# nubcico/EAV

Hardware: AMD Instinct MI355X
Metric: EEGNet training samples/sec (fwd+CE+bwd+Adam), whole job (higher is better)
Workload: dtype f32; 1 GPU; EEGNet_tor(5, Chans=30, Samples=10000, kernLength=300, F1=8, D=8, F2=64) train step on x[64,1,30,10000] fp32 per GPU (BASELINE.json configs[1]); global_batch=64, per_gpu_batch=64, parallelism=dp1

## Files before the change

### eav_amd/_lib.py

```python
from __future__ import annotations

import ctypes as C
import os

_HERE = os.path.dirname(os.path.abspath(__file__))
LIB_PATH = os.environ.get("EAV_LIB_PATH") or os.path.join(_HERE, "libeav_hip.so")


class EavError(RuntimeError):
    pass


_p = C.c_void_p
_i = C.c_int
_i64 = C.c_int64
_u64 = C.c_uint64
_f = C.c_float
_d = C.c_double

SIGNATURES = {
    "eav_reduce_partials": [_p, _i, _i64, _i, _f, _p, _p],
    "eav_bn_finalize": [_p, _i, _i, _d, _p, _p, _p, _p, _i, _f, _f, _p, _p, _p, _p, _p],
    "eav_bn_bwd_finalize": [_p, _i, _i, _d, _i, _p, _p, _p, _p, _p],
    "eav_reduce_and_bn_bwd_finalize": [_p, _i, _i64, _i, _p, _p, _i, _i, _d, _i, _p, _p, _p, _p, _p, _i, _i, _d, _i, _p, _p, _p,
                                       _p, _p],
    "eav_renorm_rows": [_p, _i, _i, _f, _p],
    "eav_renorm_rows2": [_p, _i, _i, _p, _i, _i, _f, _p],
    "eav_eegnet_step_prologue": [_p, _p, _p, _p, _p, _p, _p, _p],
    "eav_eegnet_fir_fwd": [_p, _p, _p, _p, _i, _i, _i, _i, _p],
    "eav_eegnet_fir_wgrad": [_p, _p, _p, _p, _p, _i, _i, _i, _i, _p],
    "eav_eegnet_fir_fwd_indexed": [_p, _p, _p, _p, _p, _i, _i, _i, _i, _p],
    "eav_eegnet_fir_fwd_fft": [_p, _p, _p, _p, _p, _i, _i, _i, _i, _p],
    "eav_eegnet_fir_wgrad_fft": [_p, _p, _p, _p, _p, _p, _p, _i, _i, _i, _i, _p],
    "eav_eegnet_fir_wgrad_indexed": [_p, _p, _p, _p, _p, _p, _i, _i, _i, _i, _p],
    "eav_eegnet_dw_fwd": [_p, _p, _p, _p, _p, _i, _i, _i, _p],
    "eav_eegnet_dw_fwd_pool_eval": [_p, _p, _p, _p, _p, _p, _p, _i, _i, _i, _p],
    "eav_eegnet_dw_bwd": [_p, _p, _p, _p, _p, _p, _p, _i, _i, _i, _p],
    "eav_eegnet_dw_bwd_fused": [_p, _p, _p, _p, _p, _p, _p, _p, _p, _i, _i, _i, _f, _u64, _p, _p, _p],
    "eav_eegnet_dw_bwd_fused_eval": [_p, _p, _p, _p, _p, _p, _p, _p, _p, _p, _i, _i, _i, _f, _u64, _p, _p, _p],
    "eav_bn_elu_pool_fwd": [_p, _p, _p, _i, _i, _i, _i, _f, _u64, _p, _p, _p],
    "eav_bn_elu_pool_bwd_reduce": [_p, _p, _p, _p, _i, _i, _i, _i, _f, _u64, _p, _p, _p],
    "eav_bn_elu_pool_bwd_apply": [_p, _p, _p, _p, _p, _i, _i, _i, _i, _f, _u64, _p, _p, _p],
    "eav_bn_elu_pool_bwd_eval": [_p, _p, _p, _p, _p, _i, _i, _i, _i, _f, _u64, _p, _p, _p],
    "eav_conv64_prep_weights": [_p, _p, _p, _p],
    "eav_conv64_fwd": [_p, _p, _p, _p, _i, _i, _i, _p],
    "eav_conv64_wgrad": [_p, _p, _p, _i, _i, _i, _p],
    "eav_conv64_fft_fwd": [_p, _p, _p, _p, _p, _i, _i, _i, _p],
    "eav_conv64_fft_wgrad": [_p, _p, _p, _i, _i, _p],
    "eav_dense_softmax_fwd": [_p, _p, _p, _p, _p, _i, _i, _i, _p],
    "eav_dense_softmax_bwd": [_p, _p, _p, _p, _p, _p, _p, _i, _i, _i, _p],
    "eav_ce_fwd_bwd": [_p, _p, _p, _p, _p, _p, _i, _i, _p],
    "eav_scale_by_scalar": [_p, _p, _i64, _p],
    "eav_adam_step": [_p, _p, _p, _p, _i64, _f, _f, _f, _f, _f, _i64, _i, _p, _p],
    "eav_counter_inc": [_p, _p],
    "eav_counter_inc4": [_p, _p, _p, _p, _p],
    "eav_step_begin": [_p, _p, _p, _p, _p, _p, _p, _p, _i, _p],
    "eav_gather_rows": [_p, _p, _p, _i, _i64, _p],
    "eav_gather_i64": [_p, _p, _p, _i, _p],
    "eav_gemm_f32": [_p, _p, _p, _i, _i, _i, _i, _i, _i, _i, _i, _i, _i, _i64, _i64, _i64, _i64, _i64, _i64, _f, _p,
                     _i, _p, _p, _i, _i, _p],
    "eav_gemm_f32_splitk": [_p, _p, _p, _p, _i, _i, _i, _i, _i, _i, _i, _p],
    "eav_sp_absmax": [_p, _i, _i, _i64, _p, _p],
    "eav_sp_convert": [_p, _i, _i, _i64, _p, _p, _p, _p],
    "eav_sp_convert_gelu": [_p, _i, _i, _i64, _p, _p, _p, _p],
    "eav_sp_convert_colsum": [_p, _i, _i, _i64, _p, _p, _p, _p, _p],
    "eav_layernorm_fwd_amax": [_p, _p, _p, _p, _p, _p, _i, _i, _f, _p, _p],
    "eav_layernorm_bwd_amax": [_p, _p, _p, _p, _p, _p, _i, _p, _i, _i, _p, _p],
    "eav_layernorm_bwd_planes": [_p, _p, _p, _p, _p, _p, _i, _p, _i, _i, _p, _p, _p, _p, _p, _p],
    "eav_layernorm_bwd_bound": [_p, _p, _p, _p, _p, _i, _i, _p, _p],
    "eav_gelu_bwd_amax": [_p, _p, _i64, _p, _p],
    "eav_gemm_sp": [_p, _p, _p, _p, _p, _i, _i, _i, _i, _i, _i64, _i64, _f, _p, _i, _p, _p, _i, _i, _p, _p],
    "eav_gemm_sp_x1": [_p, _p, _p, _p, _p, _i, _i, _i, _i, _i, _i64, _i64, _f, _p, _i, _p, _p, _i, _i, _p, _p],
    "eav_gemm_sp_splitk_x1": [_p, _p, _p, _p, _p, _p, _i, _i, _i, _i, _p],
    "eav_gemm_sp_splitk_x2": [_p, _p, _p, _p, _p, _p, _i, _i, _i, _i, _p],
    "eav_gemm_sp_ex": [_p, _p, _p, _p, _p, _i, _i, _i, _i, _i, _i64, _i64, _f, _p, _i, _p, _p, _i, _i, _p, _p, _p, _p, _i, _p],
    "eav_colnorm_max": [_p, _i, _i, _i64, _p, _p],
    "eav_norm_max_multi": [_p, _i, _i, _p],
    "eav_sp_bound_scale": [_p, _p, _p, _f, _p],
    "eav_gemm_sp_planes": [_p, _p, _p, _p, _p, _i, _i, _i, _i, _i, _i64, _i64, _f, _p, _i, _p, _p, _i, _i, _p, _p, _p, _p],
    "eav_layernorm_fwd_planes": [_p, _p, _p, _p, _p, _p, _p, _p, _i, _i, _f, _p],
    "eav_sp_refresh_planes": [_p, _i, _i, _i, _p],
# ... 206 lines not shown
```

### eav_amd/csrc/eav_common.h

```cpp
#pragma once
#include <hip/hip_runtime.h>
#include <stdint.h>

#define EAV_OK 0
#define EAV_EINVAL (-1)
#define EAV_ELAUNCH (-2)
#define EAV_EUNSUPPORTED (-3)

int eav_set_error(int code, const char* fmt, ...);

#define EAV_REQUIRE(cond, ...)                                   \
  do {                                                           \
    if (!(cond)) return eav_set_error(EAV_EINVAL, __VA_ARGS__);  \
  } while (0)

#define EAV_CHECK_LAUNCH(name)                                                        \
  do {                                                                                \
    hipError_t e__ = hipGetLastError();                                               \
    if (e__ != hipSuccess)                                                            \
      return eav_set_error(EAV_ELAUNCH, "%s: %s", name, hipGetErrorString(e__));      \
  } while (0)

typedef float f32x4 __attribute__((ext_vector_type(4)));
typedef float f32x16 __attribute__((ext_vector_type(16)));

static inline int cdiv(int a, int b) { return (a + b - 1) / b; }
static inline int64_t cdiv64(int64_t a, int64_t b) { return (a + b - 1) / b; }

#ifdef EAV_ABL_ELU
__device__ __forceinline__ float elu_f(float v) { return v > 0.f ? v : 0.5f * v; }
#elif defined(EAV_ELU_LIBM)
__device__ __forceinline__ float elu_f(float v) {
  const float e = expm1f(fminf(v, 0.f));
  return v <= 0.f ? e : v;
}
#else
__device__ __forceinline__ float expm1_neg(float x) {
#pragma clang fp contract(off)
  const float t = __builtin_fmaf(x, 1.4426950408889634f, 12582912.f);
  const float n = t - 12582912.f;
  float r = __builtin_fmaf(n, -0.693145751953125f, x);
  r = __builtin_fmaf(n, -1.42860682030941723212e-6f, r);
  float q = 1.394644962e-03f;
  q = __builtin_fmaf(q, r, 8.366583847e-03f);
  q = __builtin_fmaf(q, r, 4.166628048e-02f);
  q = __builtin_fmaf(q, r, 1.666654348e-01f);
  q = __builtin_fmaf(q, r, 0.5f);
  const float p = __builtin_fmaf(r * r, q, r);
  const float s = __uint_as_float((__float_as_uint(t) << 23) + 0x3f800000u);
  return __builtin_fmaf(p, s, s - 1.f);
}
__device__ __forceinline__ float elu_f(float v) {
  const float e = expm1_neg(__builtin_amdgcn_fmed3f(v, -17.5f, 0.f));
  return v <= 0.f ? e : v;
}
#endif
__device__ __forceinline__ float elu_grad_from_out(float v, float a) { return v > 0.f ? 1.f : a + 1.f; }

__device__ __forceinline__ float wave_sum(float v) {
#pragma unroll
  for (int o = 32; o > 0; o >>= 1) v += __shfl_xor(v, o, 64);
  return v;
}
__device__ __forceinline__ float half_sum(float v) {
#pragma unroll
  for (int o = 16; o > 0; o >>= 1) v += __shfl_xor(v, o, 64);
  return v;
}

template <int NV>
__device__ __forceinline__ void block_sum_256(float (&v)[NV], float* red) {
  const int lane = threadIdx.x & 63, wave = threadIdx.x >> 6;
#pragma unroll
  for (int k = 0; k < NV; ++k) {
    float s = wave_sum(v[k]);
    if (lane == 0) red[wave * NV + k] = s;
  }
  __syncthreads();
  if (threadIdx.x < NV) {
    v[0] = red[threadIdx.x] + red[NV + threadIdx.x] + red[2 * NV + threadIdx.x] + red[3 * NV + threadIdx.x];
  }
  __syncthreads();
}

#define EAV_SLOT_SHARD(i) (32 * ((i) & 63))
#define EAV_SLOT_SIGMA 2048
#define EAV_SLOT_ISIGMA 2049
#define EAV_SLOT_BMAX 2080
#define EAV_SLOT_BEXP 3104
#define EAV_SLOT_NBLK 1024
// ... 45 lines not shown
```

### eav_amd/csrc/eegnet_block.hip

```cpp
#include "eav_common.h"
#include "../../include/eav_hip.h"

namespace {

constexpr int F1 = 8, DD = 8, CHMAX = 32;

__device__ __forceinline__ void ld4(const float* p, int i, int n, bool vec, float (&v)[4]) {
  if (vec && i + 3 < n) {
    float4 a = *reinterpret_cast<const float4*>(p + i);
    v[0] = a.x; v[1] = a.y; v[2] = a.z; v[3] = a.w;
  } else {
#pragma unroll
    for (int e = 0; e < 4; ++e) v[e] = (i + e < n) ? p[i + e] : 0.f;
  }
}
__device__ __forceinline__ void ld4s(const float* p, int i, int n, bool vec, float (&v)[4]) {
  if (vec && i + 3 < n) {
    const f32x4 a = __builtin_nontemporal_load(reinterpret_cast<const f32x4*>(p + i));
    v[0] = a[0]; v[1] = a[1]; v[2] = a[2]; v[3] = a[3];
  } else {
#pragma unroll
    for (int e = 0; e < 4; ++e) v[e] = (i + e < n) ? p[i + e] : 0.f;
  }
}
// ... 184 lines not shown
  block_sum_256<2>(st, red);
  if (threadIdx.x < 2) part[(int64_t)b * 2 * CH + threadIdx.x * CH + ch] = st[0];
}

template <int P>
__global__ __launch_bounds__(256) void pool_bwd_apply_kernel(const float* __restrict__ dp,
                                                             const float* __restrict__ u,
                                                             const float* __restrict__ bn,
                                                             const float* __restrict__ m12, float* __restrict__ du,
                                                             int CH, int T, float drop_p, uint64_t seed_in,
    const uint8_t* __restrict__ mask, const uint64_t* __restrict__ seed_dev, float* __restrict__ part) {
  const uint64_t seed = dropout_seed(seed_in, seed_dev);
  __shared__ float red[8];
  const int row = blockIdx.x, ch = row % CH;
  const float mean = bn[ch], invstd = bn[CH + ch], sc = bn[2 * CH + ch], sh = bn[3 * CH + ch];
  const float m1 = m12 ? m12[ch] : 0.f, m2 = m12 ? m12[CH + ch] : 0.f;
  float st[2] = {0.f, 0.f};
  const int To = T / P;
  const float* src = u + (int64_t)row * T;
  float* dst = du + (int64_t)row * T;
  const bool vec = (T & 3) == 0;
  for (int q = threadIdx.x; q < (T + 3) / 4; q += 256) {
    const int t = 4 * q;
    const int to = t / P;
    float go = 0.f;
    if (to < To) {
      const uint64_t oi = (uint64_t)row * To + to;
      go = dp[oi] * (1.0f / P) * dropout_mult_row(drop_p, seed, mask, oi, (uint64_t)row);
    }
    float v[4], o[4];
    ld4(src, t, T, vec, v);
#pragma unroll
    for (int e = 0; e < 4; ++e) {
      const float pre = sc * v[e] + sh;
      const float g = go * elu_grad_from_out(pre, elu_f(pre));
      o[e] = sc * (g - m1 - (v[e] - mean) * invstd * m2);
      if (t + e < T) {
        st[0] += g;
        st[1] += g * ((v[e] - mean) * invstd);
      }
    }
    st4(dst, t, T, vec, o);
  }
  if (part) {
    block_sum_256<2>(st, red);
    if (threadIdx.x < 2) part[(int64_t)(row / CH) * 2 * CH + threadIdx.x * CH + ch] = st[0];
  }
}

template <int CTRL, int BANK_MASK>
__device__ __forceinline__ float dpp_f(float old, float src) {
  return __int_as_float(__builtin_amdgcn_update_dpp(__float_as_int(old), __float_as_int(src), CTRL, 0xf, BANK_MASK, false));
}

template <int CTRL, int ROW_MASK, bool BOUND>
__device__ __forceinline__ float dpp_row(float src) {
  return __int_as_float(__builtin_amdgcn_update_dpp(0, __float_as_int(src), CTRL, ROW_MASK, 0xf, BOUND));
}
__device__ __forceinline__ float wave_total_dpp(float a) {
  a += dpp_row<0x111, 0xf, true>(a);
  a += dpp_row<0x112, 0xf, true>(a);
  a += dpp_row<0x114, 0xf, true>(a);
  a += dpp_row<0x118, 0xf, true>(a);
  a += dpp_row<0x142, 0xa, false>(a);
  a += dpp_row<0x143, 0xc, false>(a);
  return __int_as_float(__builtin_amdgcn_readlane(__float_as_int(a), 63));
}

struct DwFuse {
  const float* z; const float* dp2; const float* bn2;
  float drop_p; uint64_t seed; const uint8_t* mask; const uint64_t* seed_dev;
  float* part2;
// ... 320 lines not shown
```

### eav_amd/csrc/eegnet_conv64_fft.hip

```cpp
#include <algorithm>

#include "eav_common.h"
#include "../../include/eav_hip.h"

namespace {

constexpr int NCH = 64, KT = 16, NB = 64, LV = NB - KT + 1;
typedef float v2f __attribute__((ext_vector_type(2)));
typedef __attribute__((address_space(3))) void* lds_ptr_t;
constexpr float C64[50] = {1.0f, 0.995184727f, 0.98078528f, 0.956940336f, 0.923879533f, 0.881921264f, 0.831469612f, 0.773010453f, 0.707106781f, 0.634393284f, 0.555570233f, 0.471396737f, 0.382683432f, 0.290284677f, 0.195090322f, 0.0980171403f, 0.0f, -0.0980171403f, -0.195090322f, -0.290284677f, -0.382683432f, -0.471396737f, -0.555570233f, -0.634393284f, -0.707106781f, -0.773010453f, -0.831469612f, -0.881921264f, -0.923879533f, -0.956940336f, -0.98078528f, -0.995184727f, -1.0f, -0.995184727f, -0.98078528f, -0.956940336f, -0.923879533f, -0.881921264f, -0.831469612f, -0.773010453f, -0.707106781f, -0.634393284f, -0.555570233f, -0.471396737f, -0.382683432f, -0.290284677f, -0.195090322f, -0.0980171403f, 0.0f, 0.0980171403f};
constexpr float S64[50] = {0.0f, 0.0980171403f, 0.195090322f, 0.290284677f, 0.382683432f, 0.471396737f, 0.555570233f, 0.634393284f, 0.707106781f, 0.773010453f, 0.831469612f, 0.881921264f, 0.923879533f, 0.956940336f, 0.98078528f, 0.995184727f, 1.0f, 0.995184727f, 0.98078528f, 0.956940336f, 0.923879533f, 0.881921264f, 0.831469612f, 0.773010453f, 0.707106781f, 0.634393284f, 0.555570233f, 0.471396737f, 0.382683432f, 0.290284677f, 0.195090322f, 0.0980171403f, 0.0f, -0.0980171403f, -0.195090322f, -0.290284677f, -0.382683432f, -0.471396737f, -0.555570233f, -0.634393284f, -0.707106781f, -0.773010453f, -0.831469612f, -0.881921264f, -0.923879533f, -0.956940336f, -0.98078528f, -0.995184727f, -1.0f, -0.995184727f};

__device__ __forceinline__ v2f cmul(v2f a, v2f b) { return a.xx * b + a.yy * (v2f){-b.y, b.x}; }
__device__ __forceinline__ v2f cmulc(v2f a, v2f b) { return a.xx * (v2f){b.x, -b.y} + a.yy * (v2f){b.y, b.x}; }
template <bool INV>
__device__ __forceinline__ v2f twmul(v2f a, v2f w) { return INV ? cmulc(a, w) : cmul(a, w); }
template <bool INV>
__device__ __forceinline__ v2f rot(v2f a) { return INV ? (v2f){-a.y, a.x} : (v2f){a.y, -a.x}; }

template <bool INV>
__device__ __forceinline__ void dft4(v2f& a0, v2f& a1, v2f& a2, v2f& a3) {
  const v2f t0 = a0 + a2, t1 = a0 - a2, t2 = a1 + a3, t3 = rot<INV>(a1 - a3);
  a0 = t0 + t2; a1 = t1 + t3; a2 = t0 - t2; a3 = t1 - t3;
}
// ... 10 lines not shown
}

__host__ __device__ constexpr int pos64(int k) { return 8 * (k & 7) + (k >> 3); }

template <bool INV>
__device__ __forceinline__ void fft64(v2f (&x)[64]) {
#pragma unroll
  for (int n2 = 0; n2 < 8; ++n2)
    dft8<INV>(x[n2], x[8 + n2], x[16 + n2], x[24 + n2], x[32 + n2], x[40 + n2], x[48 + n2], x[56 + n2]);
#pragma unroll
  for (int k1 = 1; k1 < 8; ++k1)
#pragma unroll
    for (int n2 = 1; n2 < 8; ++n2) x[8 * k1 + n2] = twmul<INV>(x[8 * k1 + n2], (v2f){C64[n2 * k1], -S64[n2 * k1]});
#pragma unroll
  for (int k1 = 0; k1 < 8; ++k1)
    dft8<INV>(x[8 * k1], x[8 * k1 + 1], x[8 * k1 + 2], x[8 * k1 + 3], x[8 * k1 + 4], x[8 * k1 + 5], x[8 * k1 + 6],
              x[8 * k1 + 7]);
}

struct Geo {
  int B, T, padl, nblk, npair, ncol, ncolp;
};

Geo geometry(int B, int T, int padl) {
  Geo g;
  g.B = B; g.T = T; g.padl = padl;
  g.nblk = cdiv(T, LV);
  g.npair = cdiv(g.nblk, 2);
  g.ncol = B * g.npair;
  g.ncolp = cdiv(g.ncol, 128) * 128;
  return g;
}

__global__ __launch_bounds__(64) void c64_spectra_kernel(const float* __restrict__ w, float* __restrict__ Bm0, int bwd0) {
  const int in = blockIdx.x, lane = threadIdx.x;
  const int bwd = bwd0 + blockIdx.y;
  float* Bm = Bm0 + (int64_t)blockIdx.y * 64 * 128 * 128;
  v2f x[64];
#pragma unroll
  for (int n = 0; n < 64; ++n) {
    float t = 0.f;
    if (n < KT) t = bwd ? w[((int64_t)in * NCH + lane) * KT + (KT - 1 - n)] : w[((int64_t)lane * NCH + in) * KT + n];
    x[n] = (v2f){t, 0.f};
  }
  fft64<false>(x);
#pragma unroll
  for (int m = 0; m < 64; ++m) {
    const v2f W = x[pos64(m)];
    const float gr = W.x * (1.0f / NB), gi = -W.y * (1.0f / NB);
    float* row0 = Bm + ((int64_t)m * 128 + in) * 128;
    float* row1 = Bm + ((int64_t)m * 128 + 64 + in) * 128;
    row0[lane] = gr;   row0[64 + lane] = gi;
    row1[lane] = -gi;  row1[64 + lane] = gr;
  }
}

constexpr int TS = 65;

__global__ __launch_bounds__(256) void c64_pack_fft_kernel(const float* __restrict__ in, float* __restrict__ Z, Geo g,
                                                           int vonly) {
  __shared__ float tiles[4][64 * TS];
  const int lane = threadIdx.x & 63, wave = threadIdx.x >> 6;
  float* tile = tiles[wave];
  const int nwaves = gridDim.x * 4;
  for (int col = blockIdx.x * 4 + wave; col < g.ncolp; col += nwaves) {
    if (col >= g.ncol) {
      float* dz = Z + (int64_t)col * 128 + lane;
#pragma unroll 8
      for (int m = 0; m < 64; ++m) {
        dz[(int64_t)m * g.ncolp * 128] = 0.f;
        dz[(int64_t)m * g.ncolp * 128 + 64] = 0.f;
      }
      continue;
    }
    const int b = col / g.npair, pr = col - b * g.npair;
    v2f x[64];
#pragma unroll
    for (int half = 0; half < 2; ++half) {
      const int blk = 2 * pr + half;
      const int t = blk * LV - (vonly ? 0 : g.padl) + lane;
      const bool ok = blk < g.nblk && t >= 0 && t < g.T && (!vonly || lane < LV);
      const float* src = in + (int64_t)b * NCH * g.T + t;
#pragma unroll
      for (int ch = 0; ch < NCH; ++ch) {
        const float v = ok ? src[(int64_t)ch * g.T] : 0.f;
        if (half == 0) x[ch].x = v; else x[ch].y = v;
      }
    }
#pragma unroll
    for (int half = 0; half < 2; ++half) {
#pragma unroll
      for (int ch = 0; ch < NCH; ++ch) tile[ch * TS + lane] = half == 0 ? x[ch].x : x[ch].y;
      asm volatile("s_waitcnt lgkmcnt(0)" ::: "memory");
      float r[64];
#pragma unroll
      for (int n = 0; n < 64; ++n) r[n] = tile[lane * TS + n];
      asm volatile("s_waitcnt lgkmcnt(0)" ::: "memory");
#pragma unroll
      for (int n = 0; n < 64; ++n) {
        if (half == 0) x[n].x = r[n]; else x[n].y = r[n];
      }
    }
    fft64<false>(x);
    float* dst = Z + (int64_t)col * 128 + lane;
#pragma unroll
    for (int m = 0; m < 64; ++m) {
      dst[(int64_t)m * g.ncolp * 128] = x[pos64(m)].x;
      dst[(int64_t)m * g.ncolp * 128 + 64] = x[pos64(m)].y;
    }
  }
}

constexpr int XS = 129;

#ifndef C64V_GW
#define C64V_GW 8
#endif
constexpr int GEMM_GW = C64V_GW, GEMM_AW = 8;

__global__ __launch_bounds__(256, 4) void c64_bin_gemm_kernel(const float* __restrict__ Z, const float* __restrict__ Bm,
                                                              float* __restrict__ C, int ncolp) {
  __shared__ float xs[2][32 * XS];
  const int bin = blockIdx.x, step = gridDim.y;
  const int lane = threadIdx.x & 63, wave = threadIdx.x >> 6;
  const int n = lane & 31, kk = lane >> 5;
  const int ntiles = ncolp >> 5;
  int tile = (blockIdx.y + bin) % step;
  const float* zb = Z + (int64_t)bin * ncolp * 128;
  float* cb = C + (int64_t)bin * ncolp * 128;
  const int scol = threadIdx.x >> 3, sk4 = threadIdx.x & 7;
  float4 pre[4];
  auto fetch = [&](int t) {
    const float4* src = reinterpret_cast<const float4*>(zb + ((int64_t)t * 32 + scol) * 128) + sk4;
#pragma unroll
    for (int i = 0; i < 4; ++i) pre[i] = src[8 * i];
  };
  auto commit = [&](int buf) {
    float* d = xs[buf] + scol * XS + 4 * sk4;
#pragma unroll
    for (int i = 0; i < 4; ++i) {
      d[32 * i] = pre[i].x; d[32 * i + 1] = pre[i].y; d[32 * i + 2] = pre[i].z; d[32 * i + 3] = pre[i].w;
    }
// ... 201 lines not shown
  for (int m = 0; m < 64; ++m) x[m] = *reinterpret_cast<const v2f*>(Acc + 2 * (((int64_t)m * 64 + o) * 64 + lane));
  fft64<true>(x);
#pragma unroll
  for (int k = 0; k < KT; ++k) dW[((int64_t)o * NCH + lane) * KT + k] = x[pos64(k)].x * (1.0f / NB);
}

int pack_grid(const Geo& g) { return std::max(1, std::min(512, cdiv(g.ncolp, 4))); }

}

extern "C" int64_t eav_conv64_fft_ws_floats(int B, int T) {
  const Geo g = geometry(B, T, 7);
  return (int64_t)2 * 64 * 128 * 128 + (int64_t)3 * 64 * g.ncolp * 128 + (int64_t)WCH * 64 * 128 * 128 +
         (int64_t)64 * 64 * 64 * 2;
}

extern "C" int eav_conv64_fft_nparts(int B, int T) {
  const Geo g = geometry(B, T, 7);
  return pack_grid(g) * 4;
}

extern "C" int eav_conv64_fft_fwd(const float* in, const float* w, float* out, float* stat_part, float* ws, int B, int T,
                                  int bwd, void* stream) {
  EAV_REQUIRE(in && w && out && ws && B > 0 && T > 0, "eav_conv64_fft_fwd: bad arguments");
  EAV_REQUIRE(((uintptr_t)ws & 15) == 0, "eav_conv64_fft_fwd: the workspace must be 16-byte aligned");
  const Geo g = geometry(B, T, bwd ? 8 : 7);
  EAV_REQUIRE(bwd >= 0 && bwd <= 2, "eav_conv64_fft_fwd: bwd must be 0, 1 or 2");
  hipStream_t st = (hipStream_t)stream;
  float* Bm = ws + (bwd ? (int64_t)64 * 128 * 128 : 0);
  const bool prepared = bwd == 2;
  if (bwd == 2) bwd = 1;
  float* Z = ws + (int64_t)2 * 64 * 128 * 128 + (bwd ? (int64_t)64 * g.ncolp * 128 : 0);
  float* Y = ws + (int64_t)2 * 64 * 128 * 128 + (int64_t)2 * 64 * g.ncolp * 128;
  if (!prepared) {
    hipLaunchKernelGGL(c64_spectra_kernel, dim3(NCH, bwd ? 1 : 2), dim3(64), 0, st, w, Bm, bwd);
    EAV_CHECK_LAUNCH("eav_conv64_fft_fwd(spectra)");
  }
  hipLaunchKernelGGL(c64_pack_fft_kernel, dim3(pack_grid(g)), dim3(256), 0, st, in, Z, g, 0);
  EAV_CHECK_LAUNCH("eav_conv64_fft_fwd(fft)");
  hipLaunchKernelGGL(c64_bin_gemm_kernel, dim3(64, std::min(GEMM_GW, g.ncolp / 32)), dim3(256), 0, st, Z, Bm, Y, g.ncolp);
  EAV_CHECK_LAUNCH("eav_conv64_fft_fwd(gemm)");
  hipLaunchKernelGGL(c64_ifft_unpack_kernel, dim3(pack_grid(g)), dim3(256), 0, st, Y, out, stat_part, g);
  EAV_CHECK_LAUNCH("eav_conv64_fft_fwd(ifft)");
  return EAV_OK;
}

extern "C" int eav_conv64_fft_wgrad(const float* du, float* dW, float* ws, int B, int T, void* stream) {
  EAV_REQUIRE(du && dW && ws && B > 0 && T > 0, "eav_conv64_fft_wgrad: bad arguments");
  const Geo g = geometry(B, T, 7);
  hipStream_t st = (hipStream_t)stream;
  float* Z = ws + (int64_t)2 * 64 * 128 * 128;
  float* D = Z + (int64_t)2 * 64 * g.ncolp * 128;
  float* Pp = Z + (int64_t)3 * 64 * g.ncolp * 128;
  float* Acc = Pp + (int64_t)WCH * 64 * 128 * 128;
  hipLaunchKernelGGL(c64_pack_fft_kernel, dim3(pack_grid(g)), dim3(256), 0, st, du, D, g, 1);
  EAV_CHECK_LAUNCH("eav_conv64_fft_wgrad(fft)");
  static_assert(128 % (WCH * WKB) == 0, "the padded columns split into WCH chunks of whole K-blocks");
  const int cpc = g.ncolp / WCH;
  hipLaunchKernelGGL(c64_bin_wgemm_kernel, dim3(WCH, 64), dim3(256), 0, st, D, Z, Pp, g.ncolp, cpc);
  EAV_CHECK_LAUNCH("eav_conv64_fft_wgrad(gemm)");
  hipLaunchKernelGGL(c64_wsum_kernel, dim3(64, 64), dim3(64), 0, st, Pp, Acc, WCH);
  EAV_CHECK_LAUNCH("eav_conv64_fft_wgrad(sum)");
  hipLaunchKernelGGL(c64_wfinish_kernel, dim3(NCH), dim3(64), 0, st, Acc, dW);
  EAV_CHECK_LAUNCH("eav_conv64_fft_wgrad(finish)");
  return EAV_OK;
}
```

### eav_amd/eegnet.py

```python
from __future__ import annotations

import os

import torch
import torch.nn as nn

from . import _lib
from .optim import CrossEntropyLoss, FusedAdam
from .runtime import (DeviceLoader, GraphStep, KernelFn, KernelModule, cached_workspace, eager_step,
                      gather_batch)

_PARAM_ORDER = [
    "firstConv.weight", "firstBN.weight", "firstBN.bias",
    "depthwiseConv.weight", "depthwiseBN.weight", "depthwiseBN.bias",
    "separableConv.weight", "separableBN.weight", "separableBN.bias",
    "dense.weight", "dense.bias",
]


class _Workspace:

    def __init__(self, B, C, S, klen, nb, dev):
        f = lambda *shape: torch.empty(*shape, dtype=torch.float32, device=dev)
        self.key = (B, C, S)
# ... 82 lines not shown

    def __init__(self, nb_classes, Chans=30, Samples=500, dropoutRate=0.5, kernLength=300, F1=8, D=8, F2=64,
                 norm_rate=1.0, dropoutType='Dropout'):
        super().__init__()
        self._generic = not (F1 == 8 and D == 8 and F2 == 64 and 1 <= kernLength <= 300 and 1 <= Chans <= 32)
        if not (1 <= F1 <= 16 and 1 <= D <= 8 and F1 * D <= 64 and 1 <= F2 <= 64 and 1 <= kernLength <= 1024
                and 1 <= Chans <= 256 and 1 <= nb_classes <= 16 and Samples >= 32):
            raise NotImplementedError("eav_amd.EEGNet_tor: the gfx950 kernels cover F1<=16, D<=8, F1*D<=64, F2<=64, "
                                      "kernLength<=1024, Chans<=256, nb_classes<=16, Samples>=32")
        self.dropout = nn.Dropout(dropoutRate) if dropoutType == 'Dropout' else nn.Dropout2d(dropoutRate)
        self.firstConv = nn.Conv2d(1, F1, (1, kernLength), padding='same', bias=False)
        self.firstBN = nn.BatchNorm2d(F1)
        self.elu = nn.ELU()
        self.depthwiseConv = nn.Conv2d(F1, F1 * D, (Chans, 1), groups=F1, padding=0, bias=False)
        self.depthwiseBN = nn.BatchNorm2d(F1 * D)
        self.depthwisePool = nn.AvgPool2d((1, 4))
        self.separableConv = nn.Conv2d(F1 * D, F2, (1, 16), padding='same', bias=False)
        self.separableBN = nn.BatchNorm2d(F2)
        self.separablePool = nn.AvgPool2d((1, 8))
        self.flatten = nn.Flatten()
        self.dense = nn.Linear(F2 * (Samples // 4 // 8), nb_classes)
        self.softmax = nn.Softmax(dim=1)

        self.nb_classes, self.Chans, self.Samples, self.kernLength = nb_classes, Chans, Samples, kernLength
        self.F1, self.D, self.F2 = F1, D, F2
        self.norm_rate, self.dropoutRate = float(norm_rate), float(dropoutRate)
        self.spatial_dropout = dropoutType != 'Dropout'
        self.dropout_seed = 0x0EA5EED
        self.apply_max_norm = True
        self.kernel_events = None
        self.fir_precision = "fp32"
        self.fir_algo = os.environ.get("EAV_FIR_ALGO", "auto")
        self.conv_algo = os.environ.get("EAV_CONV_ALGO", "auto")
        self._infer = False
        self._step_begin = None
        self.fused_eval = False

    def _use_fft(self):
        if self.fir_algo not in ("auto", "fft", "mfma"):
            raise ValueError(f"fir_algo {self.fir_algo!r}: expected 'auto', 'fft' or 'mfma'")
        if self.fir_algo == "mfma" or self.kernLength > _lib.plain("eav_eegnet_fir_fft_max_taps"):
            return False
        return self.fir_algo == "fft" or self.Samples >= 1408

    def _use_conv_fft(self, B):
        if self.conv_algo not in ("auto", "fft", "mfma"):
            raise ValueError(f"conv_algo {self.conv_algo!r}: expected 'auto', 'fft' or 'mfma'")
        if self.conv_algo == "mfma":
            return False
        return self.conv_algo == "fft" or B * (self.Samples // 4) >= 40000

    def forward(self, x):
        self._require_gpu(x)
        if x.dim() == 3:
            x = x.unsqueeze(1)
        if x.dim() != 4 or x.shape[1] != 1 or x.shape[2] != self.Chans or x.shape[3] != self.Samples:
            raise ValueError(f"expected input [B,1,{self.Chans},{self.Samples}], got {tuple(x.shape)}")
        self._require_same_device(x)
        x = x.contiguous().float()
        self._ensure_flat()
        self._infer = (not torch.is_grad_enabled()) and (not self.training)
        return _EEGNetFn.apply(x, self, *self._params())

    def forward_indexed(self, data, idx):
        if data.dim() != 4 or data.shape[1] != 1 or data.shape[2] != self.Chans or data.shape[3] != self.Samples or \
                not data.is_cuda or data.dtype != torch.float32 or not data.is_contiguous():
# ... 200 lines not shown
        L("eav_bn_elu_pool_bwd_reduce", P(ws.dp2), P(ws.z), b2, P(ws.part_pb), B, C2, S, 4, drop, seed1, m1, cnt, st)
        L("eav_bn_bwd_finalize", P(ws.part_pb), B, C2, float(B * S), tr, P(g["depthwiseBN.weight"]),
          P(g["depthwiseBN.bias"]), b2 + 16 * C2, b2 + 20 * C2, st)
        L("eav_bn_elu_pool_bwd_apply", P(ws.dp2), P(ws.z), b2, b2 + 16 * C2, P(ws.dz), B, C2, S, 4, drop, seed1, m1,
          cnt, st)
        b1 = P(ws.bn1)
        L("eav_spatial_bwd", P(ws.y1), P(ws.dz), b1, w2, P(ws.g1), P(ws.part_sst), P(ws.part_sw), B, C, S, F1, D, 1, st)
        L("eav_reduce_partials", P(ws.part_sw), ws.np_s, C2 * C, C2 * C, 1.0, P(g["depthwiseConv.weight"]), st)
        L("eav_bn_bwd_finalize", P(ws.part_sst), ws.np_s, F1, float(B * C * S), tr, P(g["firstBN.weight"]),
          P(g["firstBN.bias"]), b1 + 16 * F1, b1 + 20 * F1, st)
        L("eav_tconv_wgrad", P(x), P(ws.y1), P(ws.g1), b1, P(ws.part_tw), B, C, S, F1, K, st)
        L("eav_reduce_partials", P(ws.part_tw), ws.np_tw, F1 * K, F1 * K, 1.0, P(g["firstConv.weight"]), st)
        named = dict(self.named_parameters())
        return [g[k].view(named[k].shape) if named[k].requires_grad else None for k in _PARAM_ORDER]

    def _launch_backward(self, dprobs, token):
        self._check_token(token)
        if self._generic:
            return self._launch_backward_generic(dprobs)
        L, P, st = self._call, _lib.ptr, _lib.stream_ptr()
        _, x, training, drop, seed1, seed2, masks, cnt, ws, probs = self._saved
        B, C, S, K, nb = x.shape[0], self.Chans, self.Samples, self.kernLength, self.nb_classes
        T2, NF = ws.T2, ws.NF
        flat, gflat, offs = self._flat
        g = {k: gflat[offs[k][0]:offs[k][0] + offs[k][1]] for k in _PARAM_ORDER}
        w2, wd = P(self.depthwiseConv.weight), P(self.dense.weight)
        m1 = P(masks[0]) if masks is not None else None
        m2 = P(masks[1]) if masks is not None else None
        tr = int(training)

        L("eav_dense_softmax_bwd", P(dprobs), P(probs), P(ws.p3), wd, P(g["dense.weight"]), P(g["dense.bias"]),
          P(ws.dp3), B, NF, nb, st)
        b3 = P(ws.bn3)
        if training:
            L("eav_bn_elu_pool_bwd_reduce", P(ws.dp3), P(ws.u3), b3, P(ws.part_pb), B, 64, T2, 8, drop, seed2, m2, cnt, st)
            L("eav_bn_bwd_finalize", P(ws.part_pb), B, 64, float(B * T2), tr, P(g["separableBN.weight"]),
              P(g["separableBN.bias"]), b3 + 4 * 256, b3 + 4 * 320, st)
            L("eav_bn_elu_pool_bwd_apply", P(ws.dp3), P(ws.u3), b3, b3 + 4 * 256, P(ws.du3), B, 64, T2, 8, drop, seed2, m2,
              cnt, st)
        else:
            L("eav_bn_elu_pool_bwd_eval", P(ws.dp3), P(ws.u3), b3, P(ws.du3), P(ws.part_pb), B, 64, T2, 8, drop, seed2, m2,
              cnt, st)
            L("eav_bn_bwd_finalize", P(ws.part_pb), B, 64, float(B * T2), tr, P(g["separableBN.weight"]),
              P(g["separableBN.bias"]), b3 + 4 * 256, b3 + 4 * 320, st)
        if self._use_conv_fft(B):
            L("eav_conv64_fft_fwd", P(ws.du3), P(self.separableConv.weight), P(ws.dp2), None, P(ws.c64_ws), B, T2, 2, st)
        else:
            L("eav_conv64_fwd", P(ws.du3), P(ws.wTb), P(ws.dp2), None, B, T2, 8, st)
        if self._use_conv_fft(B):
            L("eav_conv64_fft_wgrad", P(ws.du3), P(g["separableConv.weight"]), P(ws.c64_ws), B, T2, st)
        else:
            L("eav_conv64_wgrad", P(ws.du3), P(ws.p2), P(ws.part_cw), B, T2, 7, st)
            L("eav_reduce_partials", P(ws.part_cw), ws.np_cw, 65536, 65536, 1.0, P(g["separableConv.weight"]), st)
        b2 = P(ws.bn2)
        b1 = P(ws.bn1)
        if training:
            L("eav_bn_elu_pool_bwd_reduce", P(ws.dp2), P(ws.z), b2, P(ws.part_pb), B, 64, S, 4, drop, seed1, m1, cnt, st)
            L("eav_bn_bwd_finalize", P(ws.part_pb), B, 64, float(B * S), tr, P(g["depthwiseBN.weight"]),
              P(g["depthwiseBN.bias"]), b2 + 4 * 256, b2 + 4 * 320, st)
            L("eav_eegnet_dw_bwd_fused", P(ws.y1), P(ws.z), P(ws.dp2), b2, b1, w2, P(ws.g1), P(ws.part_dst),
              P(ws.part_dw2), B, C, S, drop, seed1, m1, cnt, st)
        else:
            L("eav_eegnet_dw_bwd_fused_eval", P(ws.y1), P(ws.z), P(ws.dp2), b2, b1, w2, P(ws.g1), P(ws.part_dst),
              P(ws.part_dw2), P(ws.part_dw), B, C, S, drop, seed1, m1, cnt, st)
        bn2job = (None, 0, 0, 0.0, 0, None, None, None, None) if training else \
            (P(ws.part_dw), B * ws.nchunk, 64, float(B * S), tr, P(g["depthwiseBN.weight"]), P(g["depthwiseBN.bias"]),
             b2 + 4 * 256, b2 + 4 * 320)
        L("eav_reduce_and_bn_bwd_finalize", P(ws.part_dw2), B * ws.nchunk, 64 * C, 64 * C, P(g["depthwiseConv.weight"]),
          P(ws.part_dst), B * ws.nchunk, 8, float(B * C * S), tr, P(g["firstBN.weight"]), P(g["firstBN.bias"]), b1 + 4 * 32,
          b1 + 4 * 40, *bn2job, st)
        if self._use_fft():
            if ws.fft_ws is None:
                ws.fft_ws = torch.empty(_lib.plain("eav_eegnet_fir_wgrad_fft_ws_floats", B, C, S), dtype=torch.float32,
                                        device=ws.y1.device)
            xi = isinstance(x, IndexedBatch)
            L("eav_eegnet_fir_wgrad_fft", P(x.data) if xi else P(x), P(x.idx) if xi else None,
              P(ws.y1) if training else None, P(ws.g1), b1, P(ws.fft_ws), P(g["firstConv.weight"]), B, C, S, K, st)
        else:
            if isinstance(x, IndexedBatch):
                L("eav_eegnet_fir_wgrad_indexed", P(x.data), P(x.idx), P(ws.y1) if training else None, P(ws.g1), b1,
                  P(ws.part_fw), B, C, S, K, st)
            else:
                L("eav_eegnet_fir_wgrad", P(x), P(ws.y1) if training else None, P(ws.g1), b1, P(ws.part_fw), B, C, S, K,
                  st)
# ... 67 lines not shown
```

### include/eav_hip.h

```cpp
#ifndef EAV_HIP_H
#define EAV_HIP_H
#include <stdint.h>

#ifdef __cplusplus
extern "C" {
#endif

#define EAV_ABI_VERSION 3

const char* eav_last_error(void);
int eav_abi_version(void);

int eav_reduce_partials(const float* part, int nparts, int64_t stride, int n, float scale, float* out, void* stream);

int eav_bn_finalize(const float* part, int nparts, int nch, double count, const float* gamma, const float* beta,
                    float* running_mean, float* running_var, int training, float momentum, float eps, float* mean,
                    float* invstd, float* scale, float* shift, void* stream);
int eav_bn_bwd_finalize(const float* part, int nparts, int nch, double count, int training, float* dgamma,
                        float* dbeta, float* m1, float* m2, void* stream);
int eav_reduce_and_bn_bwd_finalize(const float* part, int nparts, int64_t stride, int n, float* out,
                                   const float* part_a, int nparts_a, int nch_a, double count_a, int training_a,
                                   float* dgamma_a, float* dbeta_a, float* m1_a, float* m2_a,
                                   const float* part_b, int nparts_b, int nch_b, double count_b, int training_b,
                                   float* dgamma_b, float* dbeta_b, float* m1_b, float* m2_b, void* stream);
// ... 30 lines not shown
int eav_eegnet_dw_bwd_fused(const float* y1, const float* z, const float* dp2, const float* bn2, const float* bn1,
                            const float* w2, float* g1, float* stat_part, float* w_part, int B, int C, int S,
                            float drop_p, uint64_t seed, const uint8_t* mask, const uint64_t* seed_dev, void* stream);

int eav_eegnet_dw_bwd_fused_eval(const float* y1, const float* z, const float* dp2, const float* bn2, const float* bn1,
                                 const float* w2, float* g1, float* stat_part, float* w_part, float* bn2_part, int B, int C,
                                 int S, float drop_p, uint64_t seed, const uint8_t* mask, const uint64_t* seed_dev,
                                 void* stream);

int eav_bn_elu_pool_fwd(const float* in, const float* bn, float* out, int B, int CH, int T, int P, float drop_p,
                        uint64_t seed, const uint8_t* mask, const uint64_t* seed_dev, void* stream);
int eav_bn_elu_pool_bwd_reduce(const float* dp, const float* u, const float* bn, float* part , int B,
                               int CH, int T, int P, float drop_p, uint64_t seed, const uint8_t* mask,
                               const uint64_t* seed_dev, void* stream);
int eav_bn_elu_pool_bwd_apply(const float* dp, const float* u, const float* bn, const float* m12 ,
                              float* du, int B, int CH, int T, int P, float drop_p, uint64_t seed,
                              const uint8_t* mask, const uint64_t* seed_dev, void* stream);
int eav_bn_elu_pool_bwd_eval(const float* dp, const float* u, const float* bn, float* du, float* part , int B,
                             int CH, int T, int P, float drop_p, uint64_t seed, const uint8_t* mask,
                             const uint64_t* seed_dev, void* stream);

int eav_conv64_prep_weights(const float* w , float* wT_fwd , float* wT_bwd, void* stream);
int eav_eegnet_step_prologue(const float* w, float* wT_fwd, float* wT_bwd, int64_t* c0, int64_t* c1, int64_t* c2,
                             int64_t* c3, void* stream);
int eav_conv64_ntiles(int T);
int eav_conv64_fwd_nparts(int B, int T);
int eav_conv64_fwd(const float* in, const float* wT, float* out, float* stat_part, int B, int T, int padl,
                   void* stream);
int64_t eav_conv64_fft_ws_floats(int B, int T);
int eav_conv64_fft_nparts(int B, int T);
int eav_conv64_fft_fwd(const float* in, const float* w, float* out, float* stat_part, float* ws, int B, int T, int bwd,
                       void* stream);
int eav_conv64_fft_wgrad(const float* du, float* dW, float* ws, int B, int T, void* stream);
int eav_conv64_wgrad_nparts(int B, int T);
int eav_conv64_wgrad(const float* du, const float* in, float* part, int B, int T, int padl, void* stream);

int eav_tconv_fwd_nparts(int B, int C, int S, int F1, int K);
int eav_tconv_fwd(const float* x, const float* w, float* y1, float* stat_part, int B, int C, int S, int F1, int K,
                  void* stream);
int eav_tconv_wgrad_nparts(int B, int C, int S, int F1, int K);
int eav_tconv_wgrad(const float* x, const float* y1, const float* g1, const float* bn_params, float* part, int B,
                    int C, int S, int F1, int K, void* stream);
int eav_spatial_nparts(int B, int S);
int eav_spatial_fwd(const float* y1, const float* bn1, const float* wd, float* z, float* stat_part, int B, int C,
                    int S, int F1, int D, int elu, void* stream);
int eav_spatial_bwd(const float* y1, const float* dz, const float* bn1, const float* wd, float* g1, float* stat_part,
                    float* w_part, int B, int C, int S, int F1, int D, int elu, void* stream);
int eav_dconv_fwd_nparts(int B, int T);
int eav_dconv_fwd(const float* in, const float* w, float* out, float* stat_part, int B, int Cin, int Cout, int T,
                  int K, int transposed, void* stream);
int eav_dconv_wgrad(const float* dy, const float* x, float* part, int B, int Cin, int Cout, int T, int K, void* stream);
int eav_sepconv_fwd_nparts(int B, int T);
int eav_sepconv_fwd(const float* a, const float* wdw, const float* wp, float* d3, float* z, float* stat_part, int B,
                    int C2, int F2, int T, int K2, void* stream);
int eav_pointwise_bwd_nparts(int B, int T);
int eav_pointwise_bwd(const float* du, const float* d3, const float* wp, float* dd3, float* w_part, int B, int C2,
                      int F2, int T, void* stream);
int eav_dwt_bwd(const float* dd3, const float* a, const float* wdw, float* da, float* w_part, int B, int C2, int T,
                int K2, void* stream);

int eav_dense_softmax_fwd(const float* in, const float* w, const float* bias, float* logits, float* probs, int B,
                          int NF, int NC, void* stream);
int eav_dense_softmax_bwd(const float* dout, const float* probs, const float* in, const float* w, float* dw,
                          float* dbias, float* din, int B, int NF, int NC, void* stream);
int eav_ce_fwd_bwd(const float* in, const int64_t* y, float* loss, float* din, int* ncorrect, int* bad_label, int B,
                   int NC, void* stream);
// ... 223 lines not shown
```

Measured before the change: 48840 samples/s.

## Fuse pool-backward apply into conv64 FFT backward pack and share FFTs for dgrad/wgrad

Adds a combined conv64 FFT backward entry that packs the upstream gradient once and produces both the dgrad spectrum and the wgrad spectrum in a single kernel. In training it also computes the BN/ELU/pool backward apply inline, so du3 is never written or re-read. Separately, the weight spectra kernel is folded into the forward pack kernel as extra blocks, which saves a launch. The aim is to remove a separate elementwise pass, a redundant FFT pack and several launches, at the cost of heavier kernels with more register pressure (launch bounds 256,2).

```diff
diff --git a/eav_amd/_lib.py b/eav_amd/_lib.py
--- a/eav_amd/_lib.py
+++ b/eav_amd/_lib.py
@@ -47,6 +47,7 @@
     "eav_conv64_wgrad": [_p, _p, _p, _i, _i, _i, _p],
     "eav_conv64_fft_fwd": [_p, _p, _p, _p, _p, _i, _i, _i, _p],
     "eav_conv64_fft_wgrad": [_p, _p, _p, _i, _i, _p],
+    "eav_conv64_fft_bwd": [_p, _p, _p, _p, _p, _f, _u64, _p, _p, _p, _p, _p, _i, _i, _p],
     "eav_dense_softmax_fwd": [_p, _p, _p, _p, _p, _i, _i, _i, _p],
     "eav_dense_softmax_bwd": [_p, _p, _p, _p, _p, _p, _p, _i, _i, _i, _p],
     "eav_ce_fwd_bwd": [_p, _p, _p, _p, _p, _p, _i, _i, _p],
diff --git a/eav_amd/csrc/eav_common.h b/eav_amd/csrc/eav_common.h
--- a/eav_amd/csrc/eav_common.h
+++ b/eav_amd/csrc/eav_common.h
@@ -56,6 +56,16 @@
 }
 #endif
 __device__ __forceinline__ float elu_grad_from_out(float v, float a) { return v > 0.f ? 1.f : a + 1.f; }
+
+__device__ __forceinline__ float pool_bwd_du(float v, float go, float mean, float invstd, float sc, float sh, float m1,
+                                             float m2, float& g, float& uhat) {
+#pragma clang fp contract(off)
+  const float pre = __builtin_fmaf(sc, v, sh);
+  const float eg = elu_grad_from_out(pre, elu_f(pre));
+  g = go * eg;
+  uhat = (v - mean) * invstd;
+  return sc * __builtin_fmaf(-m2, uhat, __builtin_fmaf(go, eg, -m1));
+}
 
 __device__ __forceinline__ float wave_sum(float v) {
 #pragma unroll
diff --git a/eav_amd/csrc/eegnet_block.hip b/eav_amd/csrc/eegnet_block.hip
--- a/eav_amd/csrc/eegnet_block.hip
+++ b/eav_amd/csrc/eegnet_block.hip
@@ -240,12 +240,11 @@
     ld4(src, t, T, vec, v);
 #pragma unroll
     for (int e = 0; e < 4; ++e) {
-      const float pre = sc * v[e] + sh;
-      const float g = go * elu_grad_from_out(pre, elu_f(pre));
-      o[e] = sc * (g - m1 - (v[e] - mean) * invstd * m2);
+      float g, uhat;
+      o[e] = pool_bwd_du(v[e], go, mean, invstd, sc, sh, m1, m2, g, uhat);
       if (t + e < T) {
         st[0] += g;
-        st[1] += g * ((v[e] - mean) * invstd);
+        st[1] += g * uhat;
       }
     }
     st4(dst, t, T, vec, o);
diff --git a/eav_amd/csrc/eegnet_conv64_fft.hip b/eav_amd/csrc/eegnet_conv64_fft.hip
--- a/eav_amd/csrc/eegnet_conv64_fft.hip
+++ b/eav_amd/csrc/eegnet_conv64_fft.hip
@@ -66,10 +66,8 @@
   return g;
 }
 
-__global__ __launch_bounds__(64) void c64_spectra_kernel(const float* __restrict__ w, float* __restrict__ Bm0, int bwd0) {
-  const int in = blockIdx.x, lane = threadIdx.x;
-  const int bwd = bwd0 + blockIdx.y;
-  float* Bm = Bm0 + (int64_t)blockIdx.y * 64 * 128 * 128;
+__device__ __forceinline__ void c64_spectra_wave(const float* __restrict__ w, float* __restrict__ Bm, int in, int bwd,
+                                                 int lane) {
   v2f x[64];
 #pragma unroll
   for (int n = 0; n < 64; ++n) {
@@ -91,13 +89,45 @@
 
 constexpr int TS = 65;
 
+__device__ __forceinline__ void pack_transpose(float* tile, v2f (&x)[64], int lane) {
+#pragma unroll
+  for (int half = 0; half < 2; ++half) {
+#pragma unroll
+    for (int ch = 0; ch < NCH; ++ch) tile[ch * TS + lane] = half == 0 ? x[ch].x : x[ch].y;
+    asm volatile("s_waitcnt lgkmcnt(0)" ::: "memory");
+    float r[64];
+#pragma unroll
+    for (int n = 0; n < 64; ++n) r[n] = tile[lane * TS + n];
+    asm volatile("s_waitcnt lgkmcnt(0)" ::: "memory");
+#pragma unroll
+    for (int n = 0; n < 64; ++n) {
+      if (half == 0) x[n].x = r[n]; else x[n].y = r[n];
+    }
+  }
+}
+
+__device__ __forceinline__ void pack_store(float* __restrict__ Z, const v2f (&x)[64], int col, int ncolp, int lane) {
+  float* dst = Z + (int64_t)col * 128 + lane;
+#pragma unroll
+  for (int m = 0; m < 64; ++m) {
+    dst[(int64_t)m * ncolp * 128] = x[pos64(m)].x;
+    dst[(int64_t)m * ncolp * 128 + 64] = x[pos64(m)].y;
+  }
+}
+
 __global__ __launch_bounds__(256) void c64_pack_fft_kernel(const float* __restrict__ in, float* __restrict__ Z, Geo g,
-                                                           int vonly) {
+                                                           int vonly, const float* __restrict__ w, float* __restrict__ Bm0,
+                                                           int nspec, int bwd0) {
   __shared__ float tiles[4][64 * TS];
   const int lane = threadIdx.x & 63, wave = threadIdx.x >> 6;
+  if ((int)blockIdx.x < nspec) {
+    const int job = blockIdx.x * 4 + wave, table = job >> 6;
+    c64_spectra_wave(w, Bm0 + (int64_t)table * 64 * 128 * 128, job & 63, bwd0 + table, lane);
+    return;
+  }
   float* tile = tiles[wave];
-  const int nwaves = gridDim.x * 4;
-  for (int col = blockIdx.x * 4 + wave; col < g.ncolp; col += nwaves) {
+  const int nwaves = (gridDim.x - nspec) * 4;
+  for (int col = (blockIdx.x - nspec) * 4 + wave; col < g.ncolp; col += nwaves) {
     if (col >= g.ncol) {
       float* dz = Z + (int64_t)col * 128 + lane;
 #pragma unroll 8
@@ -121,27 +151,127 @@
         if (half == 0) x[ch].x = v; else x[ch].y = v;
       }
     }
+    pack_transpose(tile, x, lane);
+    fft64<false>(x);
+    pack_store(Z, x, col, g.ncolp, lane);
+  }
+}
+
+struct DuSrc {
+  const float *dp, *u, *bn, *m12;
+  float drop_p;
+  uint64_t seed;
+  const uint8_t* mask;
+  const uint64_t* seed_dev;
+};
+constexpr int PADB = KT / 2, NPW = 9;
+
+template <bool FUSE>
+__global__ __launch_bounds__(256, 2) void c64_pack_bwd_kernel(const float* __restrict__ du, DuSrc s, float* __restrict__ Zb,
+                                                           float* __restrict__ D, Geo g) {
+  __shared__ float tiles[4][64 * TS];
+  __shared__ __attribute__((aligned(16))) float cst[FUSE ? 64 * 8 : 1];
+  const int lane = threadIdx.x & 63, wave = threadIdx.x >> 6;
+  float* tile = tiles[wave];
+  uint64_t seed = 0;
+  const int To = g.T / 8;
+  if (FUSE) {
+    seed = dropout_seed(s.seed, s.seed_dev);
+    if (threadIdx.x < 64) {
+#pragma unroll
+      for (int k = 0; k < 4; ++k) cst[threadIdx.x * 8 + k] = s.bn[k * 64 + threadIdx.x];
+      cst[threadIdx.x * 8 + 4] = s.m12[threadIdx.x];
+      cst[threadIdx.x * 8 + 5] = s.m12[64 + threadIdx.x];
+    }
+    __syncthreads();
+  }
+  const int nwaves = gridDim.x * 4;
+  for (int col = blockIdx.x * 4 + wave; col < g.ncolp; col += nwaves) {
+    if (col >= g.ncol) {
+#pragma unroll
+      for (int q = 0; q < 2; ++q) {
+        float* dz = (q ? D : Zb) + (int64_t)col * 128 + lane;
+#pragma unroll 8
+        for (int m = 0; m < 64; ++m) {
+          dz[(int64_t)m * g.ncolp * 128] = 0.f;
+          dz[(int64_t)m * g.ncolp * 128 + 64] = 0.f;
+        }
+      }
+      continue;
+    }
+    const int b = col / g.npair, pr = col - b * g.npair;
+    v2f x[64];
+    const float* in = FUSE ? s.u : du;
 #pragma unroll
     for (int half = 0; half < 2; ++half) {
-#pragma unroll
-      for (int ch = 0; ch < NCH; ++ch) tile[ch * TS + lane] = half == 0 ? x[ch].x : x[ch].y;
+      const int blk = 2 * pr + half;
+      const int t = blk * LV - PADB + lane;
+      const bool ok = blk < g.nblk && t >= 0 && t < g.T;
+      const float* src = in + (int64_t)b * NCH * g.T + t;
+#pragma unroll
+      for (int ch = 0; ch < NCH; ++ch) {
+        const float v = ok ? src[(int64_t)ch * g.T] : 0.f;
+        if (half == 0) x[ch].x = v; else x[ch].y = v;
+      }
+    }
+    if (FUSE) {
+#pragma unroll
+      for (int half = 0; half < 2; ++half) {
+        const int blk = 2 * pr + half, to0 = (blk * LV - PADB) >> 3;
+#pragma unroll
+        for (int i = 0; i < NCH * NPW / 64; ++i) {
+          const int item = i * 64 + lane, ch = item / NPW, to = to0 + item - ch * NPW;
+          float go = 0.f;
+          if (blk < g.nblk && to >= 0 && to < To) {
+            const uint64_t row = (uint64_t)b * NCH + ch, oi = row * To + to;
+            go = s.dp[oi] * (1.0f / 8) * dropout_mult_row(s.drop_p, seed, s.mask, oi, row);
+          }
+          tile[half * NCH * NPW + item] = go;
+        }
+      }
       asm volatile("s_waitcnt lgkmcnt(0)" ::: "memory");
-      float r[64];
-#pragma unroll
-      for (int n = 0; n < 64; ++n) r[n] = tile[lane * TS + n];
+      int wofs[2];
+      bool okh[2];
+#pragma unroll
+      for (int half = 0; half < 2; ++half) {
+        const int blk = 2 * pr + half, t = blk * LV - PADB + lane;
+        okh[half] = blk < g.nblk && t >= 0 && t < g.T;
+        wofs[half] = half * NCH * NPW + (t >> 3) - ((blk * LV - PADB) >> 3);
+      }
+#pragma unroll
+      for (int ch = 0; ch < NCH; ++ch) {
+        const f32x4 c0 = *reinterpret_cast<const f32x4*>(cst + ch * 8);
+        const v2f c1 = *reinterpret_cast<const v2f*>(cst + ch * 8 + 4);
+        float gd, ud;
+        const float o0 = pool_bwd_du(x[ch].x, tile[wofs[0] + ch * NPW], c0.x, c0.y, c0.z, c0.w, c1.x, c1.y, gd, ud);
+        const float o1 = pool_bwd_du(x[ch].y, tile[wofs[1] + ch * NPW], c0.x, c0.y, c0.z, c0.w, c1.x, c1.y, gd, ud);
+        x[ch].x = okh[0] ? o0 : 0.f;
+        x[ch].y = okh[1] ? o1 : 0.f;
+      }
       asm volatile("s_waitcnt lgkmcnt(0)" ::: "memory");
-#pragma unroll
-      for (int n = 0; n < 64; ++n) {
-        if (half == 0) x[n].x = r[n]; else x[n].y = r[n];
-      }
+    }
+    pack_transpose(tile, x, lane);
+    constexpr int NPK = TS - LV;
+    float yk[LV - NPK];
+#pragma unroll
+    for (int n = 0; n < LV; ++n) {
+      tile[n * 64 + lane] = x[PADB + n].x;
+      if (n < NPK) tile[(LV + n) * 64 + lane] = x[PADB + n].y;
+      else yk[n - NPK] = x[PADB + n].y;
     }
     fft64<false>(x);
-    float* dst = Z + (int64_t)col * 128 + lane;
-#pragma unroll
-    for (int m = 0; m < 64; ++m) {
-      dst[(int64_t)m * g.ncolp * 128] = x[pos64(m)].x;
-      dst[(int64_t)m * g.ncolp * 128 + 64] = x[pos64(m)].y;
-    }
+    pack_store(Zb, x, col, g.ncolp, lane);
+#pragma unroll
+    for (int n = 0; n < 64; ++n) {
+      x[n] = (v2f){0.f, 0.f};
+      if (n < LV) {
+        x[n].x = tile[n * 64 + lane];
+        x[n].y = n < NPK ? tile[(LV + n) * 64 + lane] : yk[n - NPK];
+      }
+    }
+    asm volatile("s_waitcnt lgkmcnt(0)" ::: "memory");
+    fft64<false>(x);
+    pack_store(D, x, col, g.ncolp, lane);
   }
 }
 
@@ -409,11 +539,8 @@
   if (bwd == 2) bwd = 1;
   float* Z = ws + (int64_t)2 * 64 * 128 * 128 + (bwd ? (int64_t)64 * g.ncolp * 128 : 0);
   float* Y = ws + (int64_t)2 * 64 * 128 * 128 + (int64_t)2 * 64 * g.ncolp * 128;
-  if (!prepared) {
-    hipLaunchKernelGGL(c64_spectra_kernel, dim3(NCH, bwd ? 1 : 2), dim3(64), 0, st, w, Bm, bwd);
-    EAV_CHECK_LAUNCH("eav_conv64_fft_fwd(spectra)");
-  }
-  hipLaunchKernelGGL(c64_pack_fft_kernel, dim3(pack_grid(g)), dim3(256), 0, st, in, Z, g, 0);
+  const int nspec = prepared ? 0 : (bwd ? NCH / 4 : 2 * NCH / 4);
+  hipLaunchKernelGGL(c64_pack_fft_kernel, dim3(nspec + pack_grid(g)), dim3(256), 0, st, in, Z, g, 0, w, Bm, nspec, bwd);
   EAV_CHECK_LAUNCH("eav_conv64_fft_fwd(fft)");
   hipLaunchKernelGGL(c64_bin_gemm_kernel, dim3(64, std::min(GEMM_GW, g.ncolp / 32)), dim3(256), 0, st, Z, Bm, Y, g.ncolp);
   EAV_CHECK_LAUNCH("eav_conv64_fft_fwd(gemm)");
@@ -430,7 +557,7 @@
   float* D = Z + (int64_t)2 * 64 * g.ncolp * 128;
   float* Pp = Z + (int64_t)3 * 64 * g.ncolp * 128;
   float* Acc = Pp + (int64_t)WCH * 64 * 128 * 128;
-  hipLaunchKernelGGL(c64_pack_fft_kernel, dim3(pack_grid(g)), dim3(256), 0, st, du, D, g, 1);
+  hipLaunchKernelGGL(c64_pack_fft_kernel, dim3(pack_grid(g)), dim3(256), 0, st, du, D, g, 1, nullptr, nullptr, 0, 0);
   EAV_CHECK_LAUNCH("eav_conv64_fft_wgrad(fft)");
   static_assert(128 % (WCH * WKB) == 0, "the padded columns split into WCH chunks of whole K-blocks");
   const int cpc = g.ncolp / WCH;
@@ -442,3 +569,39 @@
   EAV_CHECK_LAUNCH("eav_conv64_fft_wgrad(finish)");
   return EAV_OK;
 }
+
+extern "C" int eav_conv64_fft_bwd(const float* du, const float* dp, const float* u, const float* bn, const float* m12,
+                                  float drop_p, uint64_t seed, const uint8_t* mask, const uint64_t* seed_dev, float* dx,
+                                  float* dW, float* ws, int B, int T, void* stream) {
+  EAV_REQUIRE(dx && dW && ws && B > 0 && T > 0, "eav_conv64_fft_bwd: bad arguments");
+  EAV_REQUIRE(du || (dp && u && bn && m12), "eav_conv64_fft_bwd: neither du nor (dp, u, bn, m12)");
+  EAV_REQUIRE(du || T >= 8, "eav_conv64_fft_bwd: T %d < the pooling window", T);
+  EAV_REQUIRE(drop_p > -1.f && drop_p < 1.f, "eav_conv64_fft_bwd: dropout %f outside (-1,1)", drop_p);
+  EAV_REQUIRE(((uintptr_t)ws & 15) == 0, "eav_conv64_fft_bwd: the workspace must be 16-byte aligned");
+  const Geo g = geometry(B, T, PADB);
+  hipStream_t st = (hipStream_t)stream;
+  float* Bm = ws + (int64_t)64 * 128 * 128;
+  float* Z = ws + (int64_t)2 * 64 * 128 * 128;
+  float* Zb = Z + (int64_t)64 * g.ncolp * 128;
+  float* D = Z + (int64_t)2 * 64 * g.ncolp * 128;
+  float* Pp = Z + (int64_t)3 * 64 * g.ncolp * 128;
+  float* Acc = Pp + (int64_t)WCH * 64 * 128 * 128;
+  const DuSrc src = {dp, u, bn, m12, drop_p, seed, mask, seed_dev};
+  if (du)
+    hipLaunchKernelGGL(c64_pack_bwd_kernel<false>, dim3(pack_grid(g)), dim3(256), 0, st, du, src, Zb, D, g);
+  else
+    hipLaunchKernelGGL(c64_pack_bwd_kernel<true>, dim3(pack_grid(g)), dim3(256), 0, st, du, src, Zb, D, g);
+  EAV_CHECK_LAUNCH("eav_conv64_fft_bwd(fft)");
+  const int cpc = g.ncolp / WCH;
+  hipLaunchKernelGGL(c64_bin_wgemm_kernel, dim3(WCH, 64), dim3(256), 0, st, D, Z, Pp, g.ncolp, cpc);
+  EAV_CHECK_LAUNCH("eav_conv64_fft_bwd(wgemm)");
+  hipLaunchKernelGGL(c64_bin_gemm_kernel, dim3(64, std::min(GEMM_GW, g.ncolp / 32)), dim3(256), 0, st, Zb, Bm, D, g.ncolp);
+  EAV_CHECK_LAUNCH("eav_conv64_fft_bwd(gemm)");
+  hipLaunchKernelGGL(c64_ifft_unpack_kernel, dim3(pack_grid(g)), dim3(256), 0, st, D, dx, nullptr, g);
+  EAV_CHECK_LAUNCH("eav_conv64_fft_bwd(ifft)");
+  hipLaunchKernelGGL(c64_wsum_kernel, dim3(64, 64), dim3(64), 0, st, Pp, Acc, WCH);
+  EAV_CHECK_LAUNCH("eav_conv64_fft_bwd(sum)");
+  hipLaunchKernelGGL(c64_wfinish_kernel, dim3(NCH), dim3(64), 0, st, Acc, dW);
+  EAV_CHECK_LAUNCH("eav_conv64_fft_bwd(finish)");
+  return EAV_OK;
+}
diff --git a/eav_amd/eegnet.py b/eav_amd/eegnet.py
--- a/eav_amd/eegnet.py
+++ b/eav_amd/eegnet.py
@@ -138,6 +138,7 @@
         self.fir_precision = "fp32"
         self.fir_algo = os.environ.get("EAV_FIR_ALGO", "auto")
         self.conv_algo = os.environ.get("EAV_CONV_ALGO", "auto")
+        self.conv_fuse = os.environ.get("EAV_CONV_FUSE", "1") != "0"
         self._infer = False
         self._step_begin = None
         self.fused_eval = False
@@ -404,24 +405,27 @@
         L("eav_dense_softmax_bwd", P(dprobs), P(probs), P(ws.p3), wd, P(g["dense.weight"]), P(g["dense.bias"]),
           P(ws.dp3), B, NF, nb, st)
         b3 = P(ws.bn3)
+        fuse = bool(self.conv_fuse) and self._use_conv_fft(B)
         if training:
             L("eav_bn_elu_pool_bwd_reduce", P(ws.dp3), P(ws.u3), b3, P(ws.part_pb), B, 64, T2, 8, drop, seed2, m2, cnt, st)
             L("eav_bn_bwd_finalize", P(ws.part_pb), B, 64, float(B * T2), tr, P(g["separableBN.weight"]),
               P(g["separableBN.bias"]), b3 + 4 * 256, b3 + 4 * 320, st)
-            L("eav_bn_elu_pool_bwd_apply", P(ws.dp3), P(ws.u3), b3, b3 + 4 * 256, P(ws.du3), B, 64, T2, 8, drop, seed2, m2,
-              cnt, st)
+            if not fuse:
+                L("eav_bn_elu_pool_bwd_apply", P(ws.dp3), P(ws.u3), b3, b3 + 4 * 256, P(ws.du3), B, 64, T2, 8, drop, seed2,
+                  m2, cnt, st)
         else:
             L("eav_bn_elu_pool_bwd_eval", P(ws.dp3), P(ws.u3), b3, P(ws.du3), P(ws.part_pb), B, 64, T2, 8, drop, seed2, m2,
               cnt, st)
             L("eav_bn_bwd_finalize", P(ws.part_pb), B, 64, float(B * T2), tr, P(g["separableBN.weight"]),
               P(g["separableBN.bias"]), b3 + 4 * 256, b3 + 4 * 320, st)
-        if self._use_conv_fft(B):
+        if fuse:
+            L("eav_conv64_fft_bwd", None if training else P(ws.du3), P(ws.dp3), P(ws.u3), b3, b3 + 4 * 256, drop, seed2, m2,
+              cnt, P(ws.dp2), P(g["separableConv.weight"]), P(ws.c64_ws), B, T2, st)
+        elif self._use_conv_fft(B):
             L("eav_conv64_fft_fwd", P(ws.du3), P(self.separableConv.weight), P(ws.dp2), None, P(ws.c64_ws), B, T2, 2, st)
+            L("eav_conv64_fft_wgrad", P(ws.du3), P(g["separableConv.weight"]), P(ws.c64_ws), B, T2, st)
         else:
             L("eav_conv64_fwd", P(ws.du3), P(ws.wTb), P(ws.dp2), None, B, T2, 8, st)
-        if self._use_conv_fft(B):
-            L("eav_conv64_fft_wgrad", P(ws.du3), P(g["separableConv.weight"]), P(ws.c64_ws), B, T2, st)
-        else:
             L("eav_conv64_wgrad", P(ws.du3), P(ws.p2), P(ws.part_cw), B, T2, 7, st)
             L("eav_reduce_partials", P(ws.part_cw), ws.np_cw, 65536, 65536, 1.0, P(g["separableConv.weight"]), st)
         b2 = P(ws.bn2)
diff --git a/include/eav_hip.h b/include/eav_hip.h
--- a/include/eav_hip.h
+++ b/include/eav_hip.h
@@ -86,6 +86,9 @@
 int eav_conv64_fft_fwd(const float* in, const float* w, float* out, float* stat_part, float* ws, int B, int T, int bwd,
                        void* stream);
 int eav_conv64_fft_wgrad(const float* du, float* dW, float* ws, int B, int T, void* stream);
+int eav_conv64_fft_bwd(const float* du, const float* dp, const float* u, const float* bn, const float* m12, float drop_p,
+                       uint64_t seed, const uint8_t* mask, const uint64_t* seed_dev, float* dx, float* dW, float* ws, int B,
+                       int T, void* stream);
 int eav_conv64_wgrad_nparts(int B, int T);
 int eav_conv64_wgrad(const float* du, const float* in, float* part, int B, int T, int padl, void* stream);
 
```

Measured after the change: 49790 samples/s, median of 6. 2.0% higher.
